# TuragaLab/flybody

Measured on AMD Instinct MI355X. Metric: env steps/sec (whole node), walk_imitation 4096-batch random-action rollout, higher is better.
Workload: dtype f64

## Files before the change

### flybody_amd/csrc/fb_constraint.hpp

```cpp
#pragma once
#include "fb_types.hpp"
#include "fb_math.hpp"
#include "fb_smooth.hpp"
#include "fb_newton.hpp"

#define JIDX(side, s, r) (((r)*2 + (side))*FB_MAXCH + (s))
#define MINIMP ((real)0.0001)
#define MAXIMP ((real)0.9999)

template <typename real>
FBD real get_impedance(const real* si, real pos, real margin) {
  real s0 = fmin(MAXIMP, fmax(MINIMP, si[0])), s1 = fmin(MAXIMP, fmax(MINIMP, si[1]));
  real s2 = fmax((real)0, si[2]), s3 = fmin(MAXIMP, fmax(MINIMP, si[3])), s4 = fmax((real)1, si[4]);
  if (s0 == s1 || s2 <= FB_MINV) return (real)0.5*(s0 + s1);
  real x = fabs((pos - margin)/s2);
  if (x >= 1) return s1;
  if (x <= 0) return s0;
  real y;
  if (s4 == 1) y = x;
  else if (s4 == 2) y = (x <= s3) ? x*x/s3 : 1 - (1 - x)*(1 - x)/(1 - s3);
  else if (x <= s3) y = pow(x, s4) / pow(s3, s4 - 1);
  else y = 1 - pow(1 - x, s4) / pow(1 - s3, s4 - 1);
  return s0 + y*(s1 - s0);
}
// ... 491 lines not shown
    real detinv = fb_div((real)1, det);
    real P11 = (A22 + la)*detinv, P22 = (A11 + la)*detinv, P12 = -A12*detinv;
    v1 = -P11*b1 - P12*b2; v2 = -P12*b1 - P22*b2;
    real val = v1*v1 + v2*v2 - r*r;
    const real tolv = (sizeof(real) == 8) ? (real)1e-10 : (real)2e-6*r*r + (real)1e-10;
    if (it == 0 && sizeof(real) == 4 && la_ws && val >= tolv && *la_ws > 0) { la = *la_ws; continue; }
    if (val < tolv && (it == 0 || sizeof(real) == 8 || val > -tolv)) break;
    real deriv = -(real)2*(P11*v1*v1 + (real)2*P12*v1*v2 + P22*v2*v2);
    real delta = -fb_div(val, deriv);
    const real told = (sizeof(real) == 8) ? (real)1e-10 : (real)1e-6*la + (real)1e-10;
    if (sizeof(real) == 8) { if (delta < told) break; }
    else if (fabs(delta) < told) break;
    la += delta;
    if (la < 0) la = 0;
  }
  if (la_ws) *la_ws = la;
  res[0] = v1*dd[0]; res[1] = v2*dd[1];
  return la != 0;
}

template <typename T> struct R3 { T v0, v1, v2; };
template <bool S = false, typename T> FBD T r3_get(const R3<T>& f, int i) {
  if (S) return rdlane(f.v0, i);
  T v = (i < 64) ? f.v0 : (i < 128 ? f.v1 : f.v2);
  return rdlane(v, i & 63);
}
template <bool S = false, typename T> FBD void r3_set(R3<T>& f, int i, int lane, T v) {
  if (S) { if (lane == i) f.v0 = v; return; }
  if (lane == (i & 63)) { if (i < 64) f.v0 = v; else if (i < 128) f.v1 = v; else f.v2 = v; }
}
template <bool S = false, typename T> FBD void r3_load(R3<T>& f, const T* p, int n, int lane, T dflt) {
  f.v0 = (lane < n) ? p[lane] : dflt;
  f.v1 = (!S && lane + 64 < n) ? p[lane + 64] : dflt;
  f.v2 = (!S && lane + 128 < n) ? p[lane + 128] : dflt;
}

template <bool S, typename real, typename ARP> FBD void res_axpy(R3<double>& res, ARP AR, int i, int n, real delta, int lane) {
  const int Ti = i*(i + 1)/2;
  { int k = lane; if (k < n) res.v0 += (double)delta*(double)AR[k <= i ? Ti + k : k*(k + 1)/2 + i]; }
  if (!S) {
    { int k = lane + 64; if (k < n) res.v1 += (double)delta*(double)AR[k <= i ? Ti + k : k*(k + 1)/2 + i]; }
    { int k = lane + 128; if (k < n) res.v2 += (double)delta*(double)AR[k <= i ? Ti + k : k*(k + 1)/2 + i]; }
  }
}

template <bool S, typename real, typename ARP> FBD void res_axpy3(R3<double>& res, ARP AR, int i, int n, real e0, real e1, real e2, int lane) {
  const int T0 = i*(i + 1)/2, T1 = T0 + i + 1, T2 = T1 + i + 2;
#pragma unroll
  for (int q = 0; q < (S ? 1 : 3); q++) {
    int k = lane + 64*q;
    if (k < n) {
      int tk = k*(k + 1)/2;
      real a0 = AR[k <= i ? T0 + k : tk + i], a1 = AR[k <= i + 1 ? T1 + k : tk + i + 1], a2 = AR[k <= i + 2 ? T2 + k : tk + i + 2];
      double d = (double)e0*(double)a0 + (double)e1*(double)a1 + (double)e2*(double)a2;
      if (q == 0) res.v0 += d; else if (q == 1) res.v1 += d; else res.v2 += d;
    }
  }
}

template <typename real, typename ARP, bool S>
FB_STAGE_A int d_pgs(const DevModel<real>& M, const WS<real>& w, ARP AR, int nefc, int lane, bool sweeps = true) {
  int nv = M.nv;
  PROF_BEGIN();
  R3<real> f, rb, rR, rfr0, rfr1, rla, rdiag;
  R3<double> res;
  rla.v0 = 0; rla.v1 = 0; rla.v2 = 0;
  R3<int> rtype;
  r3_load<S>(f, w.efc_force(), nefc, lane, (real)0);
  r3_load<S>(rb, w.efc_b(), nefc, lane, (real)0);
  r3_load<S>(rR, w.efc_R(), nefc, lane, (real)0);
  r3_load<S>(rtype, w.efc_type(), nefc, lane, 0);
  rdiag.v0 = (lane < nefc) ? AR[ARIDX(lane, lane)] : (real)1;
  rdiag.v1 = (!S && lane + 64 < nefc) ? AR[ARIDX(lane + 64, lane + 64)] : (real)1;
  rdiag.v2 = (!S && lane + 128 < nefc) ? AR[ARIDX(lane + 128, lane + 128)] : (real)1;
  {
    real a0[3] = {1, 1, 1}, a1[3] = {1, 1, 1};
    for (int q = 0; q < (S ? 1 : 3); q++) {
      int r = lane + 64*q;
      a0[q] = 1; a1[q] = 1;
      if (r < nefc) { a0[q] = w.efc_s1()[r]; a1[q] = w.efc_s2()[r]; }
    }
    rfr0.v0 = a0[0]; rfr0.v1 = a0[1]; rfr0.v2 = a0[2]; rfr1.v0 = a1[0]; rfr1.v1 = a1[1]; rfr1.v2 = a1[2];
  }
  res.v0 = rb.v0; res.v1 = rb.v1; res.v2 = rb.v2;
  for (int k = 0; k < nefc; k++) {
    real fk = r3_get<S>(f, k);
    if (fk != 0) res_axpy<S>(res, AR, k, nefc, fk, lane);
  }
  if (sweeps) {
    real c = (real)0.5*(f.v0*((real)res.v0 + rb.v0) + f.v1*((real)res.v1 + rb.v1) + f.v2*((real)res.v2 + rb.v2));
    c = wave_sum(c);
    if (c > 0) { f.v0 = 0; f.v1 = 0; f.v2 = 0; res.v0 = rb.v0; res.v1 = rb.v1; res.v2 = rb.v2; }
  }
  PROF(P_CSETUP);
  R3<real> cA00, cA01, cA02, cA11, cA12, cA22, cEc, cEs, cE1, cE2, cR1, cR2, cI00;
#define FB_C3Z(name) name.v0 = 0; name.v1 = 0; name.v2 = 0;
  FB_C3Z(cA00) FB_C3Z(cA01) FB_C3Z(cA02) FB_C3Z(cA11) FB_C3Z(cA12) FB_C3Z(cA22) FB_C3Z(cEc) FB_C3Z(cEs) FB_C3Z(cE1) FB_C3Z(cE2) FB_C3Z(cR1) FB_C3Z(cR2) FB_C3Z(cI00)
#undef FB_C3Z
  if (sweeps) {
    real t[13][3];
    for (int q = 0; q < (S ? 1 : 3); q++) {
      int r = lane + 64*q;
      for (int u = 0; u < 13; u++) t[u][q] = 0;
      bool first = r < nefc && w.efc_type()[r] == CN_ELLIPTIC && w.efc_k()[r] == 0;
      if (first) {
        real a00 = AR[ARIDX(r, r)], a01 = AR[ARIDX(r + 1, r)], a02 = AR[ARIDX(r + 2, r)];
        real a11 = AR[ARIDX(r + 1, r + 1)], a12 = AR[ARIDX(r + 2, r + 1)], a22 = AR[ARIDX(r + 2, r + 2)];
        real d0 = q == 0 ? rfr0.v0 : (q == 1 ? rfr0.v1 : rfr0.v2), d1 = q == 0 ? rfr1.v0 : (q == 1 ? rfr1.v1 : rfr1.v2);
        double q11 = (double)a11*d0*d0, q22 = (double)a22*d1*d1, q12 = (double)a12*d0*d1;
        double det = q11*q22 - q12*q12;
        double m = 0.5*(q11 + q22), h = 0.5*(q11 - q22), rad = sqrt(h*h + q12*q12);
        double ev1 = m + rad, ev2 = (ev1 > 0) ? det/ev1 : 0.0;
        double vx = (h >= 0) ? h + rad : q12, vy = (h >= 0) ? q12 : rad - h;
        double vn = sqrt(vx*vx + vy*vy);
        double ec = 1, es = 0;
        if (vn > 0) { ec = vx/vn; es = vy/vn; }
        bool sing = det < 1e-10;
        t[0][q] = a00; t[1][q] = a01; t[2][q] = a02; t[3][q] = a11; t[4][q] = a12; t[5][q] = a22;
        t[6][q] = (real)ec; t[7][q] = (real)es; t[8][q] = (real)ev1; t[9][q] = (real)ev2;
        t[10][q] = sing ? (real)0 : (real)(1.0/ev1); t[11][q] = sing ? (real)0 : (real)(1.0/ev2);
        t[12][q] = (a00 >= FB_MINV) ? fb_div((real)1, a00) : (real)0;
      }
    }
#define FB_C3(name, u) name.v0 = t[u][0]; name.v1 = S ? (real)0 : t[u][1]; name.v2 = S ? (real)0 : t[u][2];
    FB_C3(cA00, 0) FB_C3(cA01, 1) FB_C3(cA02, 2) FB_C3(cA11, 3) FB_C3(cA12, 4) FB_C3(cA22, 5)
    FB_C3(cEc, 6) FB_C3(cEs, 7) FB_C3(cE1, 8) FB_C3(cE2, 9) FB_C3(cR1, 10) FB_C3(cR2, 11) FB_C3(cI00, 12)
#undef FB_C3
  }
#if defined(FB_PROFILE) && !defined(FB_EMULATE)
  long long bt_[5] = {0, 0, 0, 0, 0}, bt0_ = 0;
#define FB_BT(k) do { long long n_ = clock64(); if (k == 0) { bt_[4] += 1; } else bt_[k - 1] += n_ - bt0_; bt0_ = clock64(); } while (0)
#else
#define FB_BT(k) do {} while (0)
#endif
  real scale = (real)1 / (M.meaninertia * (real)(nv > 1 ? nv : 1));
  const int max_it = sweeps ? M.iterations : 0, max_noslip = M.noslip_iterations;
  const real tol_scaled = M.tolerance, noslip_tol = M.noslip_tolerance;
  int niter = 0;
  if (S) {
  unsigned long long m_first;
  {
    bool fst = lane < nefc && w.efc_type()[lane] == CN_ELLIPTIC && w.efc_k()[lane] == 0;
    m_first = __ballot(fst);
  }
  for (int it = 0; it < max_it; it++) {
    real improvement = 0;
    for (int i = 0; i < nefc;) {
      if (!((m_first >> i) & 1ull)) {
        real r0 = (real)rdlane(res.v0, i);
        real a = rdlane(rdiag.v0, i);
        real old = rdlane(f.v0, i);
        real fn = old - fb_div(r0, a);
        fn = fn < 0 ? (real)0 : fn;
        real del = fn - old;
        improvement -= (real)0.5*del*del*a + del*r0;
        res_axpy<true>(res, AR, i, nefc, del, lane);
        f.v0 = (lane == i) ? fn : f.v0;
        i += 1;
        continue;
      }
// ... 165 lines not shown
            }
            f1 = v1*d0; f2 = v2*d1;
          }
          FB_BT(2);
          real e0 = f0 - o0, e1 = f1 - o1, e2 = f2 - o2;
          real Ae0 = A00*e0 + A01*e1 + A02*e2, Ae1 = A01*e0 + A11*e1 + A12*e2, Ae2 = A02*e0 + A12*e1 + A22*e2;
          improvement -= (real)0.5*(e0*Ae0 + e1*Ae1 + e2*Ae2) + (e0*r0 + e1*r1 + e2*r2);
          res_axpy3<S>(res, AR, i, nefc, e0, e1, e2, lane);
          r3_set<S>(f, i, lane, f0); r3_set<S>(f, i+1, lane, f1); r3_set<S>(f, i+2, lane, f2);
          FB_BT(3);
          i += 3;
        }
      }
      niter = it + 1;
      if (improvement*scale < tol_scaled) break;
      if (it == 0) FB_SETPRIO(3);
    }
  }
  FB_SETPRIO(uniform_int(w.istate()[IS_PRIO]));
#if defined(FB_PROFILE) && !defined(FB_EMULATE)
  if (lane == 0) { long long* pp_ = (long long*)w.prof(); pp_[31] += bt_[4]; pp_[16] += bt_[0]; pp_[22] += bt_[1]; pp_[23] += bt_[2]; }
#endif
  PROF(P_PGS);
  int ncon = w.istate()[IS_NCON];
  int my_efc;
  { const int cl_ = lane < ncon ? lane : 0; const int cd_ = w.con_dim()[cl_], ce_ = w.con_efc()[cl_]; my_efc = (lane < ncon && cd_ > 1) ? ce_ : -1; }
  for (int it = 0; it < max_noslip; it++) {
    real improvement = 0;
    for (int c = 0; c < ncon; c++) {
      int i = rdlane(my_efc, c);
      if (i < 0) continue;
      real fr[2] = {r3_get<S>(rfr0, i), r3_get<S>(rfr1, i)};
      real rs[2], old[2], Rj[2];
      real fnrm = r3_get<S>(f, i);
      for (int j = 0; j < 2; j++) {
        old[j] = r3_get<S>(f, i+1+j);
        Rj[j] = r3_get<S>(rR, i+1+j);
        rs[j] = (real)r3_get<S>(res, i+1+j) - Rj[j]*old[j];
      }
      real Ac[4] = {AR[ARIDX(i+1, i+1)] - Rj[0], AR[ARIDX(i+2, i+1)],
                    AR[ARIDX(i+2, i+1)], AR[ARIDX(i+2, i+2)] - Rj[1]};
      real bc[2] = {rs[0] - (Ac[0]*old[0] + Ac[1]*old[1]), rs[1] - (Ac[2]*old[0] + Ac[3]*old[1])};
      real fq[2] = {0, 0};
      if (fnrm >= FB_MINV) {
        bool active = qcqp2(fq, Ac, bc, fr, fnrm);
        if (active) {
          real s = sqrt((fq[0]/fr[0])*(fq[0]/fr[0]) + (fq[1]/fr[1])*(fq[1]/fr[1]));
          if (s > FB_MINV) { fq[0] *= fnrm/s; fq[1] *= fnrm/s; }
        }
      }
      real del[2] = {fq[0] - old[0], fq[1] - old[1]};
      improvement -= (real)0.5*(del[0]*(Ac[0]*del[0] + Ac[1]*del[1]) + del[1]*(Ac[2]*del[0] + Ac[3]*del[1])) + del[0]*rs[0] + del[1]*rs[1];
      for (int j = 0; j < 2; j++)
        if (del[j] != 0) { res_axpy<S>(res, AR, i+1+j, nefc, del[j], lane); r3_set<S>(f, i+1+j, lane, fq[j]); }
    }
    if (improvement*scale < noslip_tol) break;
  }
  PROF(P_NOSLIP);
  if (lane < nefc) w.efc_force()[lane] = f.v0;
  if (!S) {
    if (lane + 64 < nefc) w.efc_force()[lane + 64] = f.v1;
    if (lane + 128 < nefc) w.efc_force()[lane + 128] = f.v2;
  }
  return niter;
}

template <typename real>
__device__ __forceinline__ bool d_constraint_a(const DevModel<real>& M, const WS<real>& w, int lane) {
  int nefc = w.istate()[IS_NEFC];
  int nv = M.nv;
  if (nefc == 0) {
    for (int i = lane; i < nv; i += FB_WAVE) { w.lx()[i] = 0; w.qfrc_constraint()[i] = 0; }
    if (lane == 0) w.istate()[IS_NITER] = 0;
    SYNC();
    return false;
  }
  PROF_BEGIN();
  for (int r0 = 0; r0 < nefc; r0 += FB_WAVE/4) {
    const int r = r0 + (lane >> 2), part = lane & 3, side = part >> 1, sbase = (part & 1)*(FB_MAXCH/2);
    const bool rv = r < nefc;
    const int rr = rv ? r : 0;
    real vel = 0, ja = 0, jw = 0;
    {
      int body = side ? w.efc_bB()[rr] : w.efc_bA()[rr];
      int len = rv ? (side ? w.efc_lB()[rr] : w.efc_lA()[rr]) : 0;
      const int* chp = M.body_chain + body*FB_MAXCH + sbase;
// ... 29 lines not shown
      int c = w.efc_id()[r];
      if (w.con_efc()[c] != r) continue;
      const real* fr = M.pair_friction + 5*w.con_pair()[c];
      real mu = w.efc_mu()[r];
      real j0 = w.efc_jar()[r], j1 = w.efc_jar()[r+1], j2 = w.efc_jar()[r+2];
      real U0 = j0*mu, U1 = j1*fr[0], U2 = j2*fr[1];
      real N = U0, T = sqrt(U1*U1 + U2*U2);
      real f0, f1, f2;
      if (N >= mu*T || (T <= 0 && N >= 0)) { f0 = f1 = f2 = 0; }
      else if (mu*N + T <= 0 || (T <= 0 && N < 0)) { f0 = -w.efc_D()[r]*j0; f1 = -w.efc_D()[r+1]*j1; f2 = -w.efc_D()[r+2]*j2; }
      else {
        real Dm = w.efc_D()[r] / fmax(FB_MINV, mu*mu*(1 + mu*mu));
        real NT = N - mu*T;
        f0 = -Dm*NT*mu;
        f1 = -f0/T*U1*fr[0];
        f2 = -f0/T*U2*fr[1];
      }
      w.efc_force()[r] = f0; w.efc_force()[r+1] = f1; w.efc_force()[r+2] = f2;
    }
  }
  if (!newton_any) SYNC();
  int niter;
  const int tri = nefc*(nefc + 1)/2;
  if (nefc <= LdsCfg<real>::WIDE_ROWS) {
    const bool wide = nefc > LdsCfg<real>::AR_ROWS;
    const bool k_in_slot = newton && !wide && 2*tri <= LdsCfg<real>::AR_ELEMS + FB_MAXNV;
    const bool park = wide || (newton && !k_in_slot);
    if (park) {
      for (int i = lane; i < M.nM; i += FB_WAVE) w.qLD()[i] = w.lLD[i];
      SYNC();
    }
    if (wide) {
      const real* src = w.AR();
      for (int i = lane; i < tri; i += FB_WAVE) w.lLD[i] = src[i];
      SYNC();
    }
    const FB_LDS real* arp = wide ? (const FB_LDS real*)w.lLD : (const FB_LDS real*)w.lAR();
    if (newton) {
      const WS<real> wc = w;
      constexpr int MT = 1, MR = 2;
      if (k_in_slot && nefc <= FB_NEWTON_NT) niter = d_newton<real, const FB_LDS real*, FB_LDS real*, MT>(M, wc, arp, w.lAR() + tri, nefc, lane);
      else if (k_in_slot) niter = d_newton<real, const FB_LDS real*, FB_LDS real*, MR>(M, wc, arp, w.lAR() + tri, nefc, lane);
      else if (!wide) niter = d_newton<real, const FB_LDS real*, FB_LDS real*, MR>(M, wc, arp, w.lLD, nefc, lane);
      else if (2*tri <= FB_LDS_SCRATCH + LdsCfg<real>::AR_ELEMS) niter = d_newton<real, const FB_LDS real*, FB_LDS real*, MR>(M, wc, arp, w.lLD + tri, nefc, lane);
      else niter = d_newton<real, const FB_LDS real*, real*, MR>(M, wc, arp, w.AR() + tri, nefc, lane);
      SYNC();
    }
    if (!newton || M.noslip_iterations > 0) { const int it2 = d_pgs<real, const FB_LDS real*, true>(M, w, arp, nefc, lane, !newton); if (!newton) niter = it2; }
    if (park) {
      SYNC();
      for (int i = lane; i < M.nM; i += FB_WAVE) w.lLD[i] = w.qLD()[i];
      SYNC();
    }
  }
  else if (nefc <= 64) {
    if (newton) {
      const WS<real> wc = w;
      niter = d_newton<real, const real*, real*, 2>(M, wc, (const real*)w.AR(), w.AR() + tri, nefc, lane);
      SYNC();
    }
    if (!newton || M.noslip_iterations > 0) { const int it2 = d_pgs<real, const real*, true>(M, w, (const real*)w.AR(), nefc, lane, !newton); if (!newton) niter = it2; }
  }
  else if (newton_any) {
    const WS<real> wc = w;
    niter = d_newton_wide<real>(M, wc, nefc, lane);
    SYNC();
    if (M.noslip_iterations > 0) d_pgs<real, const real*, false>(M, w, (const real*)w.AR(), nefc, lane, false);
  }
  else niter = d_pgs<real, const real*, false>(M, w, (const real*)w.AR(), nefc, lane);
  if (lane == 0) {
    w.istate()[IS_NITER] = niter;
    int wbits = (niter >= M.iterations ? WARN_SOLVER_MAXITER : 0);
    if (wbits) { atomicOr(w.istate() + IS_WARN, wbits); atomicOr(w.istate() + IS_WARN_EVER, wbits); }
  }
  SYNC();
  if (nefc <= FB_WAVE) {
    real fr = (lane < nefc) ? w.efc_force()[lane] : (real)0;
    int eA = (lane < nefc) ? w.efc_eA()[lane] : -1, eB = (lane < nefc) ? w.efc_eB()[lane] : -1;
    int dep[2], nd[2]; real acc[2] = {0, 0};
#pragma unroll
    for (int q = 0; q < 2; q++) { int i = lane + q*FB_WAVE; bool has = i < nv; dep[q] = has ? M.dof_depth[i] : 0; nd[q] = has ? M.dof_ndesc[i] : -1; }
    for (int r0 = 0; r0 < nefc; r0 += 8) {
      real ja[8][2], jb[8][2];
#pragma unroll
      for (int u = 0; u < 8; u++) {
        const int r = min(r0 + u, nefc - 1);
#pragma unroll
        for (int q = 0; q < 2; q++) { ja[u][q] = w.efc_J()[JIDX(0, dep[q], r)]; jb[u][q] = w.efc_J()[JIDX(1, dep[q], r)]; }
      }
#pragma unroll
      for (int u = 0; u < 8; u++) {
        if (r0 + u < nefc) {
          const int r = r0 + u;
          const real f = rdlane(fr, r);
          const int ea = rdlane(eA, r), eb = rdlane(eB, r);
#pragma unroll
          for (int q = 0; q < 2; q++) {
            const int i = lane + q*FB_WAVE;
            const bool onA = nd[q] >= 0 && ea >= i && ea <= i + nd[q], onB = nd[q] >= 0 && eb >= i && eb <= i + nd[q];
            if (onA) acc[q] += ja[u][q]*f;
// ... 39 lines not shown
```

### flybody_amd/csrc/fb_engine.hip

```cpp
#ifdef FB_EMULATE
#include "emu/hip_emu.hpp"
#else
#include <hip/hip_runtime.h>
#endif
#include <algorithm>
#include <cmath>
#include <cstdio>
#include <cstdlib>
#include <cstring>
#include <map>
#include <stdexcept>
#include <string>
#include <vector>
#if defined(FB_EMULATE) && defined(FB_STATS)
extern "C" { long long fb_stats[64]; }
#endif

#include "../../include/flybody_engine.h"
#include "fb_step.hpp"
#include "fb_ik.hpp"
#include "fb_inverse.hpp"

static thread_local std::string g_err;
static int fail(const std::string& s) { g_err = s; return -1; }
// ... 835 lines not shown

template <typename real>
static int build_devmodel(fb_batch* b, const fb_model* m, DevModel<real>& M) {
  memset(&M, 0, sizeof(M));
  M.nq = m->nq; M.nv = m->nv; M.nbody = m->nbody; M.njnt = m->njnt; M.ngeom = m->ngeom; M.nsite = m->nsite;
  M.nu = m->nu; M.na = m->na; M.ntendon = m->ntendon; M.npair = m->npair; M.nM = m->nM; M.nsubstep = m->nsubstep;
  M.nobsjnt = m->nobsjnt; M.napp = m->napp; M.nforce = m->nforce; M.ntouch = m->ntouch;
  M.site_thorax = m->i("sensor_site_thorax")[0]; M.nadh = (int)m->adh_act.size();
  M.iterations = m->i("opt_iterations")[0]; M.noslip_iterations = m->i("opt_noslip_iterations")[0];
  M.solver = (m->has("opt_solver", 1) && m->i("opt_solver")[0] == FB_SOLVER_PGS) ? FB_SOLVER_PGS : FB_SOLVER_NEWTON;
  M.timestep = (real)m->d("opt_timestep")[0]; M.control_timestep = (real)m->d("opt_control_timestep")[0];
  for (int k = 0; k < 3; k++) M.grav[k] = (real)m->d("opt_gravity")[k];
  M.density = (real)m->d("opt_density")[0]; M.viscosity = (real)m->d("opt_viscosity")[0];
  M.impratio = (real)m->d("opt_impratio")[0]; M.tolerance = (real)m->d("opt_tolerance")[0];
  {
    std::vector<double> rb; const double* r_ = m->d("geom_rbound");
    for (int g = 0; g < m->ngeom; g++) if (r_[g] > 0) rb.push_back(r_[g]);
    std::sort(rb.begin(), rb.end());
    M.vl_delta = (rb.empty() || m->npair <= 4*FB_WAVE) ? (real)0 : (real)(FB_VL_SCALE*rb[rb.size()/2]);
    { const char* e_ = getenv("FB_NO_NEIGHBOUR_LIST"); if (e_ && e_[0] == '1') M.vl_delta = 0; }
  }
  M.ar_entry_lanes = 1;
  { const char* e_ = getenv("FB_NO_AR_ENTRY_LANES"); if (e_ && e_[0] == '1') M.ar_entry_lanes = 0; }
  M.noslip_tolerance = (real)m->d("opt_noslip_tolerance")[0]; M.meaninertia = (real)m->d("stat_meaninertia")[0];
  M.totalmass = (real)m->totalmass;
  size_t c;
#define UI(field, name) { const int* s_ = m->i(name, &c); if (upload_i(b, s_, c, &M.field)) return -1; }
#define UV(field, vec) { if (upload_i(b, m->vec.data(), m->vec.size(), &M.field)) return -1; }
#define UD(field, name) { const double* s_ = m->d(name, &c); if (upload<real>(b, s_, c, &M.field)) return -1; }
  UI(body_parent, "body_parent") UI(body_dofadr, "body_dofadr")
  UV(body_nsub, body_nsub) UV(body_depth, body_depth) UV(body_chlen, body_chlen) UV(body_chain, body_chain) UV(body_common, body_common)
  UI(jnt_type, "jnt_type") UI(jnt_qposadr, "jnt_qposadr") UI(jnt_dofadr, "jnt_dofadr") UI(jnt_bodyid, "jnt_bodyid") UI(jnt_limited, "jnt_limited")
  UI(dof_bodyid, "dof_bodyid") UI(dof_jntid, "dof_jntid") UI(dof_Madr, "dof_Madr") UV(dof_depth, dof_depth)
  UV(dof_ndesc, dof_ndesc) UV(body_fluid_geom, body_fluid_geom) UV(sens_body, sens_body) M.nsensbody = (int)m->sens_body.size();
  UV(dof_jump, dof_jump) UV(dof_vbef, dof_vbef) UV(body_veldof, body_veldof)
  UV(dof_cl, dof_cl) UV(dof_gen, dof_gen) UV(gen_k, gen_k) UV(gen_m, gen_m) UV(fwd_tab, fwd_tab) UV(fwd_pack, fwd_pack) UV(fac_w, fac_w) UV(fac_band, fac_band) UV(fac_dof, fac_dof) M.ntrunk = m->ntrunk; M.prefix_split = m->prefix_split;
  { int dmax = 0, d2 = 1 << 20; for (int bq = 1; bq < m->nbody; bq++) { dmax = std::max(dmax, m->body_depth[bq]); if (bq >= FB_WAVE) d2 = std::min(d2, m->body_depth[bq]); } M.fk_dmax = dmax; M.fk2_dlo = d2; }
  { int cm = 0; for (int bq = 0; bq < m->nbody; bq++) cm = std::max(cm, m->body_chlen[bq]); M.chmax = cm; }
  {
    std::vector<int> second(FB_WAVE, -1);
    bool ok = m->nbody > FB_WAVE && m->nbody <= 2*FB_WAVE && getenv("FB_NO_FK_MERGE") == nullptr;
    for (int bq = FB_WAVE; ok && bq < m->nbody; bq++) {
      int pick = -1;
      for (int l = 0; l < FB_WAVE && pick < 0; l++) if (second[l] < 0 && (l == 0 || m->body_depth[l] < m->body_depth[bq])) pick = l;
      if (pick < 0) ok = false; else second[pick] = bq;
    }
// ... 809 lines not shown
```

### flybody_amd/csrc/fb_newton.hpp

```cpp
#pragma once
#include "fb_types.hpp"
#include "fb_math.hpp"
#include "fb_smooth.hpp"

#define FB_NEWTON_LS_MAX 20
#define FB_NEWTON_MAXROWS 64
#define FB_NEWTON_NT 16
#define FB_NEWTON_F32_FLOOR 1e-10
enum { FB_SOLVER_PGS = 0, FB_SOLVER_CG = 1, FB_SOLVER_NEWTON = 2 };

#define FB_NEWTON_ATTR __device__ FB_NOINLINE

template <typename real> struct NwConst { int k; bool ell; real D, sqD, s0, s1, s2, mu, Dm, g1; };
template <typename real> struct NwRow { real f, cost, fr0, fr1, fr2, fc0, fc1, fc2; };

template <typename real>
FBD void nw_update(const NwConst<real>& c, real jb0, real jb1, real jb2, NwRow<real>& o) {
  const real jo = c.k == 0 ? jb0 : (c.k == 1 ? jb1 : jb2);
  const real U0 = jb0*c.s0, U1 = jb1*c.s1, U2 = jb2*c.s2;
#ifndef FB_EMULATE
  const real TT = U1*U1 + U2*U2;
  const real Tr = TT > 0 ? fb_rsqrt(TT) : (real)0;
  const real N = U0, T = TT*Tr;
#else
// ... 390 lines not shown
#pragma unroll
            for (int I = 0; I < NB; I++) {
              const real Lip = nw_lane(T[I][Ip][q], 4*ti + P)*invp;
              const bool prow = (I == Ip) && ti == pr;
              const real Lm = prow ? (real)0 : Lip;
#pragma unroll
              for (int J = Ip; J < NB; J++)
#pragma unroll
                for (int s = 0; s < 4; s++) T[I][J][s] -= Lm*rp[J][s];
              yv[I] -= Lm*yp;
              if (I == Ip) invd[I] = prow ? invp : invd[I];
            }
          }
        }
      }
    }
  }
  real zr = 0;
#pragma unroll
  for (int I = 0; I < NB; I++) { const real zI = nw_lane(yv[I]*invd[I], 4*(my_ci & 15)); zr = (my_ci >> 4) == I ? zI : zr; }
  SYNC();
  return mine ? zr : (real)0;
}
template <typename real, typename ARP, typename KP, int MODE = 0>
FB_NEWTON_ATTR int d_newton(const DevModel<real>& M_, const WS<real>& w_, ARP AR, KP K, int nefc, int lane) {
  const DevModel<real>& M = as_constant(M_); const WS<real> w = ws_uniform(w_, M);
  const int n = nefc;
  const bool on = lane < n;
#if defined(FB_PROFILE) && !defined(FB_EMULATE)
  long long nwp_[7] = {0, 0, 0, 0, 0, 0, 0}, nwt_ = clock64(), nwc_[2] = {0, 0};
#define NW_PROF(k) do { long long n_ = clock64(); nwp_[k] += n_ - nwt_; nwt_ = clock64(); } while (0)
#define NW_COUNT(k) nwc_[k]++
#else
#define NW_PROF(k) do {} while (0)
#define NW_COUNT(k) do {} while (0)
#endif
  const int type = on ? w.efc_type()[lane] : CN_LIMIT;
  const int kblk = on ? w.efc_k()[lane] : 0;
  const real R = on ? w.efc_R()[lane] : (real)1;
  const real Dl = on ? w.efc_D()[lane] : (real)0;
  const real b = on ? w.efc_b()[lane] : (real)0;
  const real jarw = on ? w.efc_jar()[lane] : (real)0;
  const real mul = on ? w.efc_mu()[lane] : (real)0;
  const real s1l = on ? w.efc_s1()[lane] : (real)1, s2l = on ? w.efc_s2()[lane] : (real)1;
  NwConst<real> c;
  c.ell = type == CN_ELLIPTIC;
  c.k = c.ell ? kblk : 0;
  const int base = lane - c.k;
// ... 298 lines not shown
    NwRow<real> o2 = o;
    real tb0 = jb0, tb1 = jb1, tb2 = jb2;
    for (int kls = 0; kls <= FB_NEWTON_LS_MAX; kls++) {
      NW_COUNT(1);
      if (kls > 0) { tb0 = jb0 + alpha*Ab0; tb1 = jb1 + alpha*Ab1; tb2 = jb2 + alpha*Ab2; nw_update(c, tb0, tb1, tb2, o2); }
      const real wv = o2.fc0*Ab0 + o2.fc1*Ab1 + o2.fc2*Ab2;
      const real g = lAd + alpha*dAd - NW_SUM(o2.f*Adl);
      const real h = dAd + NW_SUM(wv*wv);
      if (kls == 0) { g0 = g; if (!(g0 < 0) || !(h > FB_MINV)) break; alpha = -fb_div(g0, h); continue; }
      if (fabs(g) <= (real)0.01*fabs(g0) || kls == FB_NEWTON_LS_MAX) break;
      if (g < 0) lo = alpha; else hi = alpha;
      real an = (h > FB_MINV) ? alpha - fb_div(g, h) : (real)-1;
      if (!(an > lo) || (hi >= 0 && !(an < hi))) an = (hi < 0) ? 2*alpha : (real)0.5*(lo + hi);
      alpha = an;
    }
    NW_PROF(6); NW_COUNT(0);
    if (!(alpha > 0)) break;
    lam += alpha*dl; jb0 = tb0; jb1 = tb1; jb2 = tb2;
    o = o2;
    niter = it + 1;
    if (-g0*alpha*scale < tol) break;
  }
  if (on) w.efc_force()[lane] = o.f;
  if (tile) { if (on) ARw[lane*(lane + 1)/2 + lane] = ar_diag; SYNC_LDS(); }
  if (n > FB_NEWTON_NT) FB_SETPRIO(uniform_int(w.istate()[IS_PRIO]));
#if defined(FB_PROFILE) && !defined(FB_EMULATE)
  if (lane == 0) { long long* pp_ = (long long*)w.prof(); for (int k_ = 0; k_ < 7; k_++) pp_[32 + k_] += nwp_[k_]; pp_[39] += nwc_[0]; pp_[40] += nwc_[1]; pp_[41] += 1; }
#endif
  return niter;
}
```

### flybody_amd/csrc/fb_smooth.hpp

```cpp
#pragma once
#include "fb_types.hpp"
#include "fb_math.hpp"

#ifdef FB_EMULATE
#define SYNC() __syncthreads()
#else
#define SYNC() do { __builtin_amdgcn_fence(__ATOMIC_SEQ_CST, "wavefront"); __builtin_amdgcn_wave_barrier(); } while (0)
#endif
#ifdef FB_EMULATE
#define SYNC_LDS() __syncthreads()
#else
#define SYNC_LDS() do { asm volatile("s_waitcnt lgkmcnt(0)" ::: "memory"); __builtin_amdgcn_wave_barrier(); } while (0)
#endif
#if defined(FB_PROFILE) && !defined(FB_EMULATE)
#define PROF_BEGIN() long long prof_t_ = clock64()
#define PROF_RESET() prof_t_ = clock64()
#define PROF(id) do { long long now_ = clock64(); if (lane == 0) { long long* pp_ = (long long*)w.prof(); pp_[id] += now_ - prof_t_; } prof_t_ = clock64(); } while (0)
#else
#define PROF_BEGIN() do {} while (0)
#define PROF_RESET() do {} while (0)
#define PROF(id) do {} while (0)
#endif
enum { P_KIN = 0, P_COMPOS, P_CRB, P_FACTOR, P_COLL, P_MAKEC, P_PROJ, P_VEL, P_ACT, P_ACC, P_CSETUP, P_PGS, P_NOSLIP, P_CFIN, P_SENS, P_EULER, P_EPI };

// ... 627 lines not shown
  if (lane == 0) { long long* pp_ = (long long*)w.prof(); pp_[16] += fp_[0]; pp_[18] += fp_[1]; pp_[22] += fp_[2]; pp_[23] += fp_[3]; pp_[24] += fp_[4]; }
#endif
  PROF(P_FACTOR);
  PROF_RESET();
  d_factor_tail(M, w_, qM, diag_add, hscale, RM, x, lane);
}

template <typename real>
FB_STAGE_FS void d_factor_tail(const DevModel<real>& M_, const WS<real>& w_, const FB_GLOBAL real* qM, const FB_GLOBAL real* diag_add, real hscale,
                              FB_LDS real* RM, FB_LDS real* x, int lane) {
  const DevModel<real>& M = as_constant(M_); const WS<real> w = ws_uniform(w_, M);
  qM = uniform_p(qM); diag_add = uniform_p(diag_add); RM = uniform_p(RM); x = uniform_p(x);
  PROF_BEGIN();
  const int nv = uniform_int(M.nv), nT = uniform_int(M.ntrunk);
  int fd[2], jt[2];
#pragma unroll
  for (int q = 0; q < 2; q++) {
    const int j = fac_dof(w, lane, q);
    bool has = j >= 0;
    jt[q] = has ? j : 0;
    int dp = has ? w.ldepth()[j] : 31, mj = has ? w.lmadr()[j] : 0;
    fd[q] = ((mj - dp*(dp + 1)/2) & 0x1fff) | (dp << 13);
  }
  int fw[FB_FSLOT];
#pragma unroll
  for (int s = 0; s < FB_FSLOT; s++) fw[s] = M.fac_w[s*FB_WAVE + lane];
  real S[FB_NTT], xt[FB_MAXTRUNK];
#pragma unroll
  for (int e = 0; e < FB_NTT; e++) S[e] = 0;
#pragma unroll
  for (int a = 0; a < FB_MAXTRUNK; a++) xt[a] = 0;
#pragma unroll
  for (int q = 0; q < 2; q++) {
    int dep = FW_DEP(fd[q]);
    if (dep != 31) {
      int row = FW_BASE(fd[q]) + dep*(dep + 1)/2;
      real dk = RM[row], col[FB_MAXTRUNK], xk = x[jt[q]];
#pragma unroll
      for (int a = 0; a < FB_MAXTRUNK; a++) col[a] = (a < nT) ? RM[row + dep - a] : (real)0;
#pragma unroll
      for (int a = 0; a < FB_MAXTRUNK; a++) {
        real ca = col[a]*dk;
        xt[a] += ca*xk;
#pragma unroll
        for (int b2 = 0; b2 <= a; b2++) S[a*(a + 1)/2 + b2] += ca*col[b2];
      }
    }
  }
#pragma unroll
  for (int a = 0; a < FB_MAXTRUNK; a++) xt[a] = (a < nT) ? x[a] - wave_sum(xt[a]) : (real)0;
  {
    real m0[FB_NTT], dadd[FB_MAXTRUNK];
#pragma unroll
    for (int a = 0; a < FB_MAXTRUNK; a++) {
      dadd[a] = diag_add ? hscale*diag_add[a < nT ? a : 0] : (real)0;
#pragma unroll
      for (int b2 = 0; b2 <= a; b2++) m0[a*(a + 1)/2 + b2] = qM[a < nT ? a*(a + 1)/2 + (a - b2) : 0];
    }
#pragma unroll
    for (int a = 0; a < FB_MAXTRUNK; a++)
#pragma unroll
      for (int b2 = 0; b2 <= a; b2++) {
        const int e = a*(a + 1)/2 + b2;
        real m = m0[e];
        if (a == b2) m += dadd[a];
        S[e] = (a < nT) ? m - wave_sum(S[e]) : (real)0;
      }
  }
  SYNC();
#pragma unroll
  for (int h = 0; h < 2; h++) {
    constexpr int HS = FB_FSLOT/2;
    real v[HS], dd[HS]; int adr[HS];
#pragma unroll
    for (int s = 0; s < HS; s++) {
      int wd = fw[h*HS + s], dep = FW_DEP(wd);
      bool ok = dep != 31;
      int ad = ok ? FW_BASE(wd) + dep*(dep + 1)/2 : 0;
      adr[s] = ok ? ad + FW_E(wd) : FB_LDS_SCRATCH - 1;
      v[s] = RM[adr[s]]; dd[s] = RM[ad];
    }
#pragma unroll
    for (int s = 0; s < HS; s++) RM[adr[s]] = v[s]*dd[s];
  }
  real Lt[FB_NTT];
#pragma unroll
  for (int k = FB_MAXTRUNK - 1; k >= 0; k--) {
    if (k < nT) {
      real Dk = S[k*(k + 1)/2 + k], Di = fb_inv(Dk);
      if (lane == 0) RM[k*(k + 1)/2] = Di;
#pragma unroll
      for (int a = 0; a < k; a++) {
        real Lka = S[k*(k + 1)/2 + a]*Di;
        Lt[k*(k + 1)/2 + a] = Lka;
        if (lane == 0) RM[k*(k + 1)/2 + (k - a)] = Lka;
// ... 384 lines not shown
```

### flybody_amd/csrc/fb_types.hpp

```cpp
#pragma once
#ifdef FB_EMULATE
#include "emu/hip_emu.hpp"
#else
#include <hip/hip_runtime.h>
#endif
#include <stdint.h>

#if defined(FB_EMULATE) && defined(FB_STATS)
extern "C" { extern long long fb_stats[64]; }
#define FB_STAT(k) (fb_stats[k]++)
#else
#define FB_STAT(k) do {} while (0)
#endif

#define FB_WAVE 64
#define FB_EPB 4
#define FB_MAXCH 20
#define FB_MAXGEN 16
#define FB_LDS_SCRATCH 1216
#define FB_LGEN 6
#define FB_BODYREC 40
#define FB_MAXTRUNK 6
#define FB_FSLOT 18
#define FB_FGEN 2
// ... 64 lines not shown

#define FB_WS_INT(X) \
  X(istate, IS_N) X(prof, 2*FB_NPROF) X(con_pair, FB_MAXCON_) X(con_efc, FB_MAXCON_) X(con_dim, FB_MAXCON_) X(cand, 2*FB_MAXCON_ + 64) \
  X(efc_type, FB_MAXEFC_) X(efc_id, FB_MAXEFC_) X(efc_bA, FB_MAXEFC_) X(efc_bB, FB_MAXEFC_) X(efc_lA, FB_MAXEFC_) X(efc_lB, FB_MAXEFC_) \
  X(efc_k, FB_MAXEFC_)  X(efc_eA, FB_MAXEFC_) X(efc_eB, FB_MAXEFC_)  \
  X(vl_list, FB_VLMAX)

struct WSOff {
#define X(name, n) uint32_t name;
  FB_WS_REAL(X)
  FB_WS_INT(X)
#undef X
  uint32_t nreal, nint;
};

template <typename real>
struct DevModel {
  int nq, nv, nbody, njnt, ngeom, nsite, nu, na, ntendon, npair, nM, nsubstep;
  int nobsjnt, napp, nforce, ntouch, site_thorax, nadh;
  int iterations, noslip_iterations, solver;
  real timestep, control_timestep, grav[3], density, viscosity, impratio, tolerance, noslip_tolerance, meaninertia, totalmass;
  real vl_delta;
  int ar_entry_lanes;
  GP<const int> body_parent, body_dofadr, body_nsub, body_depth;
  GP<const int> body_chlen;
  GP<const int> body_chain;
  GP<const int> body_common;
  GP<const int> jnt_type, jnt_qposadr, jnt_dofadr, jnt_bodyid, jnt_limited;
  GP<const int> dof_bodyid, dof_jntid, dof_Madr, dof_depth;
  GP<const int> dof_ndesc;
  int nlevel;
  GP<const int> dof_cl;
  GP<const int> dof_gen;
  GP<const int> gen_k, gen_m;
  GP<const int> fwd_tab;
  GP<const int> fwd_pack;
  GP<const int> fac_w;
  GP<const int> fac_band;
  GP<const int> fac_dof;
  int ntrunk;
  int prefix_split;
  int chmax;
  int fk_dmax, fk2_dlo;
  const int* fk_second;
  GP<const int> geom_type, geom_bodyid, site_bodyid, site_type;
  GP<const int> tendon_adr, tendon_num;
// ... 88 lines not shown
```

Measured before the change: 854,200.

## Hand Newton solution to noslip in registers and split noslip out of PGS

Pulls the noslip pass out of d_pgs into its own routine. When Newton runs in f64 with noslip enabled, Newton now returns each lane's force and residual in registers, so noslip skips rebuilding the residual from AR and skips a sync plus a global reload of efc_force. Per-contact AR and friction values are preloaded once per lane, and paired residual updates are fused into one pass over AR. It also moves the factor-weight loads later, builds trunk M entries with one lane per element, and splits the scatter into three chunks, which trades register pressure against more rounds.

```diff
diff --git a/flybody_amd/csrc/fb_constraint.hpp b/flybody_amd/csrc/fb_constraint.hpp
--- a/flybody_amd/csrc/fb_constraint.hpp
+++ b/flybody_amd/csrc/fb_constraint.hpp
@@ -537,7 +537,8 @@
 template <typename T> struct R3 { T v0, v1, v2; };
 template <bool S = false, typename T> FBD T r3_get(const R3<T>& f, int i) {
   if (S) return rdlane(f.v0, i);
-  T v = (i < 64) ? f.v0 : (i < 128 ? f.v1 : f.v2);
+  const T a = f.v0, b = f.v1, c = f.v2;
+  T v = (i < 64) ? a : (i < 128 ? b : c);
   return rdlane(v, i & 63);
 }
 template <bool S = false, typename T> FBD void r3_set(R3<T>& f, int i, int lane, T v) {
@@ -573,8 +574,115 @@
   }
 }
 
+template <bool S, typename real, typename ARP> FBD void res_axpy2(R3<double>& res, ARP AR, int i, int n, real d0, real d1, int lane) {
+  const int T0 = i*(i + 1)/2, T1 = T0 + i + 1;
+#pragma unroll
+  for (int q = 0; q < (S ? 1 : 3); q++) {
+    int k = lane + 64*q;
+    if (k < n) {
+      int tk = k*(k + 1)/2;
+      real a0 = AR[k <= i ? T0 + k : tk + i], a1 = AR[k <= i + 1 ? T1 + k : tk + i + 1];
+      double r = q == 0 ? res.v0 : (q == 1 ? res.v1 : res.v2);
+      r = (d0 != 0) ? r + (double)d0*(double)a0 : r;
+      r = (d1 != 0) ? r + (double)d1*(double)a1 : r;
+      if (q == 0) res.v0 = r; else if (q == 1) res.v1 = r; else res.v2 = r;
+    }
+  }
+}
+template <bool S, typename T> FBD T r3_lane(const R3<T>& f, int idx) {
+  const T a = __shfl(f.v0, idx & 63, 64);
+  if (S) return a;
+  const T b = __shfl(f.v1, idx & 63, 64), c = __shfl(f.v2, idx & 63, 64);
+  return idx < 64 ? a : (idx < 128 ? b : c);
+}
+
+template <bool S, typename real, typename ARP>
+FBD void d_noslip(const DevModel<real>& M, const WS<real>& w, ARP AR, int nefc, int lane, R3<real>& f, R3<double>& res,
+                  const R3<real>& rR, const R3<real>& rfr0, const R3<real>& rfr1) {
+  PROF_BEGIN();
+  const int max_noslip = M.noslip_iterations;
+  const real noslip_tol = M.noslip_tolerance;
+  const real scale = (real)1 / (M.meaninertia * (real)(M.nv > 1 ? M.nv : 1));
+  int ncon = w.istate()[IS_NCON];
+  int my_efc;
+  { const int cl_ = lane < ncon ? lane : 0; const int cd_ = w.con_dim()[cl_], ce_ = w.con_efc()[cl_]; my_efc = (lane < ncon && cd_ > 1) ? ce_ : -1; }
+  real kA0 = 0, kA1 = 0, kA3 = 0;
+  const int ib = my_efc < 0 ? 0 : my_efc;
+  const real kF0 = r3_lane<S>(rfr0, ib), kF1 = r3_lane<S>(rfr1, ib), kR0 = r3_lane<S>(rR, ib + 1), kR1 = r3_lane<S>(rR, ib + 2);
+  if (my_efc >= 0) {
+    const real a11 = AR[ARIDX(ib+1, ib+1)], a21 = AR[ARIDX(ib+2, ib+1)], a22 = AR[ARIDX(ib+2, ib+2)];
+    kA0 = a11 - kR0; kA1 = a21; kA3 = a22 - kR1;
+  }
+  for (int it = 0; it < max_noslip; it++) {
+    real improvement = 0;
+    for (int c = 0; c < ncon; c++) {
+      int i = rdlane(my_efc, c);
+      if (i < 0) continue;
+      real fr[2] = {rdlane(kF0, c), rdlane(kF1, c)};
+      real rs[2], old[2], Rj[2] = {rdlane(kR0, c), rdlane(kR1, c)};
+      real fnrm = r3_get<S>(f, i);
+      for (int j = 0; j < 2; j++) {
+        old[j] = r3_get<S>(f, i+1+j);
+        rs[j] = (real)r3_get<S>(res, i+1+j) - Rj[j]*old[j];
+      }
+      real Ac[4] = {rdlane(kA0, c), rdlane(kA1, c), 0, rdlane(kA3, c)};
+      Ac[2] = Ac[1];
+      real bc[2] = {rs[0] - (Ac[0]*old[0] + Ac[1]*old[1]), rs[1] - (Ac[2]*old[0] + Ac[3]*old[1])};
+      real fq[2] = {0, 0};
+      if (fnrm >= FB_MINV) {
+        bool active = qcqp2(fq, Ac, bc, fr, fnrm);
+        if (active) {
+          real s = sqrt((fq[0]/fr[0])*(fq[0]/fr[0]) + (fq[1]/fr[1])*(fq[1]/fr[1]));
+          if (s > FB_MINV) { fq[0] *= fnrm/s; fq[1] *= fnrm/s; }
+        }
+      }
+      real del[2] = {fq[0] - old[0], fq[1] - old[1]};
+      improvement -= (real)0.5*(del[0]*(Ac[0]*del[0] + Ac[1]*del[1]) + del[1]*(Ac[2]*del[0] + Ac[3]*del[1])) + del[0]*rs[0] + del[1]*rs[1];
+      res_axpy2<S>(res, AR, i+1, nefc, del[0], del[1], lane);
+      for (int j = 0; j < 2; j++)
+        if (del[j] != 0) r3_set<S>(f, i+1+j, lane, fq[j]);
+    }
+    if (improvement*scale < noslip_tol) break;
+  }
+  PROF(P_NOSLIP);
+}
+
+template <bool S, typename real, typename ARP>
+FBD void noslip_load(const DevModel<real>& M, const WS<real>& w, ARP AR, int nefc, int lane, R3<real>& f, R3<double>& res,
+                     R3<real>& rR, R3<real>& rfr0, R3<real>& rfr1) {
+  PROF_BEGIN();
+  R3<real> rb;
+  r3_load<S>(f, w.efc_force(), nefc, lane, (real)0);
+  r3_load<S>(rb, w.efc_b(), nefc, lane, (real)0);
+  r3_load<S>(rR, w.efc_R(), nefc, lane, (real)0);
+  r3_load<S>(rfr0, w.efc_s1(), nefc, lane, (real)1);
+  r3_load<S>(rfr1, w.efc_s2(), nefc, lane, (real)1);
+  res.v0 = rb.v0; res.v1 = rb.v1; res.v2 = rb.v2;
+  for (int k = 0; k < nefc; k++) {
+    real fk = r3_get<S>(f, k);
+    if (fk != 0) res_axpy<S>(res, AR, k, nefc, fk, lane);
+  }
+  PROF(P_CSETUP);
+}
+template <bool S, typename real>
+FBD void noslip_store(const WS<real>& w, int nefc, int lane, const R3<real>& f) {
+  if (lane < nefc) w.efc_force()[lane] = f.v0;
+  if (!S) {
+    if (lane + 64 < nefc) w.efc_force()[lane + 64] = f.v1;
+    if (lane + 128 < nefc) w.efc_force()[lane + 128] = f.v2;
+  }
+}
 template <typename real, typename ARP, bool S>
-FB_STAGE_A int d_pgs(const DevModel<real>& M, const WS<real>& w, ARP AR, int nefc, int lane, bool sweeps = true) {
+FB_STAGE_A void d_noslip_mem(const DevModel<real>& M, const WS<real>& w, ARP AR, int nefc, int lane) {
+  R3<real> f, rR, rfr0, rfr1;
+  R3<double> res;
+  noslip_load<S>(M, w, AR, nefc, lane, f, res, rR, rfr0, rfr1);
+  d_noslip<S>(M, w, AR, nefc, lane, f, res, rR, rfr0, rfr1);
+  noslip_store<S>(w, nefc, lane, f);
+}
+
+template <typename real, typename ARP, bool S>
+FB_STAGE_A int d_pgs(const DevModel<real>& M, const WS<real>& w, ARP AR, int nefc, int lane) {
   int nv = M.nv;
   PROF_BEGIN();
   R3<real> f, rb, rR, rfr0, rfr1, rla, rdiag;
@@ -602,7 +710,7 @@
     real fk = r3_get<S>(f, k);
     if (fk != 0) res_axpy<S>(res, AR, k, nefc, fk, lane);
   }
-  if (sweeps) {
+  {
     real c = (real)0.5*(f.v0*((real)res.v0 + rb.v0) + f.v1*((real)res.v1 + rb.v1) + f.v2*((real)res.v2 + rb.v2));
     c = wave_sum(c);
     if (c > 0) { f.v0 = 0; f.v1 = 0; f.v2 = 0; res.v0 = rb.v0; res.v1 = rb.v1; res.v2 = rb.v2; }
@@ -612,7 +720,7 @@
 #define FB_C3Z(name) name.v0 = 0; name.v1 = 0; name.v2 = 0;
   FB_C3Z(cA00) FB_C3Z(cA01) FB_C3Z(cA02) FB_C3Z(cA11) FB_C3Z(cA12) FB_C3Z(cA22) FB_C3Z(cEc) FB_C3Z(cEs) FB_C3Z(cE1) FB_C3Z(cE2) FB_C3Z(cR1) FB_C3Z(cR2) FB_C3Z(cI00)
 #undef FB_C3Z
-  if (sweeps) {
+  {
     real t[13][3];
     for (int q = 0; q < (S ? 1 : 3); q++) {
       int r = lane + 64*q;
@@ -649,8 +757,8 @@
 #define FB_BT(k) do {} while (0)
 #endif
   real scale = (real)1 / (M.meaninertia * (real)(nv > 1 ? nv : 1));
-  const int max_it = sweeps ? M.iterations : 0, max_noslip = M.noslip_iterations;
-  const real tol_scaled = M.tolerance, noslip_tol = M.noslip_tolerance;
+  const int max_it = M.iterations;
+  const real tol_scaled = M.tolerance;
   int niter = 0;
   if (S) {
   unsigned long long m_first;
@@ -862,46 +970,8 @@
   if (lane == 0) { long long* pp_ = (long long*)w.prof(); pp_[31] += bt_[4]; pp_[16] += bt_[0]; pp_[22] += bt_[1]; pp_[23] += bt_[2]; }
 #endif
   PROF(P_PGS);
-  int ncon = w.istate()[IS_NCON];
-  int my_efc;
-  { const int cl_ = lane < ncon ? lane : 0; const int cd_ = w.con_dim()[cl_], ce_ = w.con_efc()[cl_]; my_efc = (lane < ncon && cd_ > 1) ? ce_ : -1; }
-  for (int it = 0; it < max_noslip; it++) {
-    real improvement = 0;
-    for (int c = 0; c < ncon; c++) {
-      int i = rdlane(my_efc, c);
-      if (i < 0) continue;
-      real fr[2] = {r3_get<S>(rfr0, i), r3_get<S>(rfr1, i)};
-      real rs[2], old[2], Rj[2];
-      real fnrm = r3_get<S>(f, i);
-      for (int j = 0; j < 2; j++) {
-        old[j] = r3_get<S>(f, i+1+j);
-        Rj[j] = r3_get<S>(rR, i+1+j);
-        rs[j] = (real)r3_get<S>(res, i+1+j) - Rj[j]*old[j];
-      }
-      real Ac[4] = {AR[ARIDX(i+1, i+1)] - Rj[0], AR[ARIDX(i+2, i+1)],
-                    AR[ARIDX(i+2, i+1)], AR[ARIDX(i+2, i+2)] - Rj[1]};
-      real bc[2] = {rs[0] - (Ac[0]*old[0] + Ac[1]*old[1]), rs[1] - (Ac[2]*old[0] + Ac[3]*old[1])};
-      real fq[2] = {0, 0};
-      if (fnrm >= FB_MINV) {
-        bool active = qcqp2(fq, Ac, bc, fr, fnrm);
-        if (active) {
-          real s = sqrt((fq[0]/fr[0])*(fq[0]/fr[0]) + (fq[1]/fr[1])*(fq[1]/fr[1]));
-          if (s > FB_MINV) { fq[0] *= fnrm/s; fq[1] *= fnrm/s; }
-        }
-      }
-      real del[2] = {fq[0] - old[0], fq[1] - old[1]};
-      improvement -= (real)0.5*(del[0]*(Ac[0]*del[0] + Ac[1]*del[1]) + del[1]*(Ac[2]*del[0] + Ac[3]*del[1])) + del[0]*rs[0] + del[1]*rs[1];
-      for (int j = 0; j < 2; j++)
-        if (del[j] != 0) { res_axpy<S>(res, AR, i+1+j, nefc, del[j], lane); r3_set<S>(f, i+1+j, lane, fq[j]); }
-    }
-    if (improvement*scale < noslip_tol) break;
-  }
-  PROF(P_NOSLIP);
-  if (lane < nefc) w.efc_force()[lane] = f.v0;
-  if (!S) {
-    if (lane + 64 < nefc) w.efc_force()[lane + 64] = f.v1;
-    if (lane + 128 < nefc) w.efc_force()[lane + 128] = f.v2;
-  }
+  if (M.noslip_iterations > 0) d_noslip<S>(M, w, AR, nefc, lane, f, res, rR, rfr0, rfr1);
+  noslip_store<S>(w, nefc, lane, f);
   return niter;
 }
 
@@ -977,6 +1047,9 @@
   if (!newton_any) SYNC();
   int niter;
   const int tri = nefc*(nefc + 1)/2;
+  const bool hand_ok = sizeof(real) == 8 && uniform_int(M.solver_handover) != 0;
+  const bool noslip = uniform_int(M.noslip_iterations) > 0;
+  bool fr_reg = false; real fr = 0;
   if (nefc <= LdsCfg<real>::WIDE_ROWS) {
     const bool wide = nefc > LdsCfg<real>::AR_ROWS;
     const bool k_in_slot = newton && !wide && 2*tri <= LdsCfg<real>::AR_ELEMS + FB_MAXNV;
@@ -994,14 +1067,29 @@
     if (newton) {
       const WS<real> wc = w;
       constexpr int MT = 1, MR = 2;
-      if (k_in_slot && nefc <= FB_NEWTON_NT) niter = d_newton<real, const FB_LDS real*, FB_LDS real*, MT>(M, wc, arp, w.lAR() + tri, nefc, lane);
-      else if (k_in_slot) niter = d_newton<real, const FB_LDS real*, FB_LDS real*, MR>(M, wc, arp, w.lAR() + tri, nefc, lane);
-      else if (!wide) niter = d_newton<real, const FB_LDS real*, FB_LDS real*, MR>(M, wc, arp, w.lLD, nefc, lane);
-      else if (2*tri <= FB_LDS_SCRATCH + LdsCfg<real>::AR_ELEMS) niter = d_newton<real, const FB_LDS real*, FB_LDS real*, MR>(M, wc, arp, w.lLD + tri, nefc, lane);
-      else niter = d_newton<real, const FB_LDS real*, real*, MR>(M, wc, arp, w.AR() + tri, nefc, lane);
-      SYNC();
-    }
-    if (!newton || M.noslip_iterations > 0) { const int it2 = d_pgs<real, const FB_LDS real*, true>(M, w, arp, nefc, lane, !newton); if (!newton) niter = it2; }
+      NwOut<real> r;
+      FB_LDS real* const kl = k_in_slot ? w.lAR() + tri : (wide ? w.lLD + tri : w.lLD);
+      if (k_in_slot && nefc <= FB_NEWTON_NT) r = d_newton<real, const FB_LDS real*, FB_LDS real*, MT, true>(M, wc, arp, kl, nefc, lane);
+      else if (!wide || 2*tri <= FB_LDS_SCRATCH + LdsCfg<real>::AR_ELEMS) r = d_newton<real, const FB_LDS real*, FB_LDS real*, MR, true>(M, wc, arp, kl, nefc, lane);
+      else r = d_newton<real, const FB_LDS real*, real*, MR, true>(M, wc, arp, w.AR() + tri, nefc, lane);
+      niter = r.niter;
+      if (!hand_ok) SYNC();
+      fr = r.f;
+      if (noslip) {
+        R3<real> f, rR, rfr0, rfr1;
+        R3<double> res;
+        if (hand_ok) {
+          f.v0 = r.f; f.v1 = 0; f.v2 = 0; res.v0 = (double)r.res; res.v1 = 0; res.v2 = 0;
+          r3_load<true>(rR, w.efc_R(), nefc, lane, (real)0); r3_load<true>(rfr0, w.efc_s1(), nefc, lane, (real)1); r3_load<true>(rfr1, w.efc_s2(), nefc, lane, (real)1);
+        }
+        else noslip_load<true>(M, w, arp, nefc, lane, f, res, rR, rfr0, rfr1);
+        d_noslip<true>(M, w, arp, nefc, lane, f, res, rR, rfr0, rfr1);
+        noslip_store<true>(w, nefc, lane, f);
+        fr = f.v0;
+      }
+      fr_reg = hand_ok;
+    }
+    else niter = d_pgs<real, const FB_LDS real*, true>(M, w, arp, nefc, lane);
     if (park) {
       SYNC();
       for (int i = lane; i < M.nM; i += FB_WAVE) w.lLD[i] = w.qLD()[i];
@@ -1011,16 +1099,17 @@
   else if (nefc <= 64) {
     if (newton) {
       const WS<real> wc = w;
-      niter = d_newton<real, const real*, real*, 2>(M, wc, (const real*)w.AR(), w.AR() + tri, nefc, lane);
+      niter = d_newton<real, const real*, real*, 2>(M, wc, (const real*)w.AR(), w.AR() + tri, nefc, lane).niter;
       SYNC();
-    }
-    if (!newton || M.noslip_iterations > 0) { const int it2 = d_pgs<real, const real*, true>(M, w, (const real*)w.AR(), nefc, lane, !newton); if (!newton) niter = it2; }
+      if (noslip) d_noslip_mem<real, const real*, true>(M, w, (const real*)w.AR(), nefc, lane);
+    }
+    else niter = d_pgs<real, const real*, true>(M, w, (const real*)w.AR(), nefc, lane);
   }
   else if (newton_any) {
     const WS<real> wc = w;
     niter = d_newton_wide<real>(M, wc, nefc, lane);
     SYNC();
-    if (M.noslip_iterations > 0) d_pgs<real, const real*, false>(M, w, (const real*)w.AR(), nefc, lane, false);
+    if (noslip) d_noslip_mem<real, const real*, false>(M, w, (const real*)w.AR(), nefc, lane);
   }
   else niter = d_pgs<real, const real*, false>(M, w, (const real*)w.AR(), nefc, lane);
   if (lane == 0) {
@@ -1028,9 +1117,9 @@
     int wbits = (niter >= M.iterations ? WARN_SOLVER_MAXITER : 0);
     if (wbits) { atomicOr(w.istate() + IS_WARN, wbits); atomicOr(w.istate() + IS_WARN_EVER, wbits); }
   }
-  SYNC();
+  if (!fr_reg) SYNC();
   if (nefc <= FB_WAVE) {
-    real fr = (lane < nefc) ? w.efc_force()[lane] : (real)0;
+    if (!fr_reg) fr = (lane < nefc) ? w.efc_force()[lane] : (real)0;
     int eA = (lane < nefc) ? w.efc_eA()[lane] : -1, eB = (lane < nefc) ? w.efc_eB()[lane] : -1;
     int dep[2], nd[2]; real acc[2] = {0, 0};
 #pragma unroll
diff --git a/flybody_amd/csrc/fb_engine.hip b/flybody_amd/csrc/fb_engine.hip
--- a/flybody_amd/csrc/fb_engine.hip
+++ b/flybody_amd/csrc/fb_engine.hip
@@ -881,6 +881,8 @@
   }
   M.ar_entry_lanes = 1;
   { const char* e_ = getenv("FB_NO_AR_ENTRY_LANES"); if (e_ && e_[0] == '1') M.ar_entry_lanes = 0; }
+  M.solver_handover = 1;
+  { const char* e_ = getenv("FB_NO_SOLVER_HANDOVER"); if (e_ && e_[0] == '1') M.solver_handover = 0; }
   M.noslip_tolerance = (real)m->d("opt_noslip_tolerance")[0]; M.meaninertia = (real)m->d("stat_meaninertia")[0];
   M.totalmass = (real)m->totalmass;
   size_t c;
diff --git a/flybody_amd/csrc/fb_newton.hpp b/flybody_amd/csrc/fb_newton.hpp
--- a/flybody_amd/csrc/fb_newton.hpp
+++ b/flybody_amd/csrc/fb_newton.hpp
@@ -436,8 +436,13 @@
   SYNC();
   return mine ? zr : (real)0;
 }
-template <typename real, typename ARP, typename KP, int MODE = 0>
-FB_NEWTON_ATTR int d_newton(const DevModel<real>& M_, const WS<real>& w_, ARP AR, KP K, int nefc, int lane) {
+template <typename real> struct NwOut { int niter; real f, res; };
+template <typename real, bool HAND> FBD bool nw_hands_over(const DevModel<real>& M) {
+  if (sizeof(real) != 8 || !HAND) return false;
+  return uniform_int(M.solver_handover) != 0 && uniform_int(M.noslip_iterations) > 0;
+}
+template <typename real, typename ARP, typename KP, int MODE = 0, bool HAND = false>
+FB_NEWTON_ATTR NwOut<real> d_newton(const DevModel<real>& M_, const WS<real>& w_, ARP AR, KP K, int nefc, int lane) {
   const DevModel<real>& M = as_constant(M_); const WS<real> w = ws_uniform(w_, M);
   const int n = nefc;
   const bool on = lane < n;
@@ -782,10 +787,13 @@
     if (-g0*alpha*scale < tol) break;
   }
   if (on) w.efc_force()[lane] = o.f;
+  NwOut<real> out;
+  out.niter = niter; out.f = on ? o.f : (real)0; out.res = 0;
+  if (nw_hands_over<real, HAND>(M)) { const real Af = amul(out.f); out.res = on ? (b + Af) + R*out.f : (real)0; }
   if (tile) { if (on) ARw[lane*(lane + 1)/2 + lane] = ar_diag; SYNC_LDS(); }
   if (n > FB_NEWTON_NT) FB_SETPRIO(uniform_int(w.istate()[IS_PRIO]));
 #if defined(FB_PROFILE) && !defined(FB_EMULATE)
   if (lane == 0) { long long* pp_ = (long long*)w.prof(); for (int k_ = 0; k_ < 7; k_++) pp_[32 + k_] += nwp_[k_]; pp_[39] += nwc_[0]; pp_[40] += nwc_[1]; pp_[41] += 1; }
 #endif
-  return niter;
+  return out;
 }
diff --git a/flybody_amd/csrc/fb_smooth.hpp b/flybody_amd/csrc/fb_smooth.hpp
--- a/flybody_amd/csrc/fb_smooth.hpp
+++ b/flybody_amd/csrc/fb_smooth.hpp
@@ -673,9 +673,6 @@
     int dp = has ? w.ldepth()[j] : 31, mj = has ? w.lmadr()[j] : 0;
     fd[q] = ((mj - dp*(dp + 1)/2) & 0x1fff) | (dp << 13);
   }
-  int fw[FB_FSLOT];
-#pragma unroll
-  for (int s = 0; s < FB_FSLOT; s++) fw[s] = M.fac_w[s*FB_WAVE + lane];
   real S[FB_NTT], xt[FB_MAXTRUNK];
 #pragma unroll
   for (int e = 0; e < FB_NTT; e++) S[e] = 0;
@@ -698,30 +695,35 @@
       }
     }
   }
+  int fw[FB_FSLOT];
+#pragma unroll
+  for (int s = 0; s < FB_FSLOT; s++) fw[s] = M.fac_w[s*FB_WAVE + lane];
 #pragma unroll
   for (int a = 0; a < FB_MAXTRUNK; a++) xt[a] = (a < nT) ? x[a] - wave_sum(xt[a]) : (real)0;
   {
-    real m0[FB_NTT], dadd[FB_MAXTRUNK];
-#pragma unroll
-    for (int a = 0; a < FB_MAXTRUNK; a++) {
-      dadd[a] = diag_add ? hscale*diag_add[a < nT ? a : 0] : (real)0;
-#pragma unroll
-      for (int b2 = 0; b2 <= a; b2++) m0[a*(a + 1)/2 + b2] = qM[a < nT ? a*(a + 1)/2 + (a - b2) : 0];
-    }
+    static_assert(FB_NTT + FB_MAXTRUNK <= FB_WAVE, "one lane per trunk entry of M and per damping term");
+    int ta = 0;
+#pragma unroll
+    for (int k = 1; k < FB_MAXTRUNK; k++) ta = (lane >= k*(k + 1)/2) ? k : ta;
+    const int tb = lane - ta*(ta + 1)/2;
+    const int da = lane - FB_NTT;
+    real mt = (real)0;
+    if (lane < FB_NTT) mt = qM[ta < nT ? ta*(ta + 1)/2 + (ta - tb) : 0];
+    else if (da < FB_MAXTRUNK && diag_add) mt = hscale*diag_add[da < nT ? da : 0];
 #pragma unroll
     for (int a = 0; a < FB_MAXTRUNK; a++)
 #pragma unroll
       for (int b2 = 0; b2 <= a; b2++) {
         const int e = a*(a + 1)/2 + b2;
-        real m = m0[e];
-        if (a == b2) m += dadd[a];
+        real m = rdlane(mt, e);
+        if (a == b2) m += rdlane(mt, FB_NTT + a);
         S[e] = (a < nT) ? m - wave_sum(S[e]) : (real)0;
       }
   }
   SYNC();
 #pragma unroll
-  for (int h = 0; h < 2; h++) {
-    constexpr int HS = FB_FSLOT/2;
+  for (int h = 0; h < 3; h++) {
+    constexpr int HS = FB_FSLOT/3;
     real v[HS], dd[HS]; int adr[HS];
 #pragma unroll
     for (int s = 0; s < HS; s++) {
diff --git a/flybody_amd/csrc/fb_types.hpp b/flybody_amd/csrc/fb_types.hpp
--- a/flybody_amd/csrc/fb_types.hpp
+++ b/flybody_amd/csrc/fb_types.hpp
@@ -110,6 +110,7 @@
   real timestep, control_timestep, grav[3], density, viscosity, impratio, tolerance, noslip_tolerance, meaninertia, totalmass;
   real vl_delta;
   int ar_entry_lanes;
+  int solver_handover;
   GP<const int> body_parent, body_dofadr, body_nsub, body_depth;
   GP<const int> body_chlen;
   GP<const int> body_chain;
```

Result: faster. 872,900 (median of 6 runs) (+2.2%).
